# ORNL-Fusion/graph_framework

Measured on AMD Instinct MI355X. Metric: ray-steps/sec on xrays_bench cold-plasma; achieved HBM GB/s vs peak, higher is better.
Workload: dtype f64

## Files before the change

graph_framework_amd/build.py:

```python
import glob
import os
import subprocess

from . import _lib

HIPCC = os.environ.get("HIPCC", "/opt/rocm/bin/hipcc")
KERNEL_FLAGS = ["-O3", "-ffp-contract=off", "-fno-slp-vectorize", "--offload-arch=gfx950"]


def build_library(force=False):
    csrc = os.path.join(_lib.HERE, "csrc")
    sources = glob.glob(os.path.join(csrc, "*")) + glob.glob(os.path.join(_lib.HERE, "..", "include", "*.h"))
    newest = max(os.path.getmtime(s) for s in sources)
    programs = [os.path.join(_lib.HERE, name) for name in ("xrays_bench", "solver_check", "korc_push")]
    sources.append(os.path.join(_lib.HERE, "gf_workflow.hpp"))
    newest = max(os.path.getmtime(s) for s in sources)
    if (force or not os.path.exists(_lib.LIB_PATH) or os.path.getmtime(_lib.LIB_PATH) < newest
            or any(not os.path.exists(p) or os.path.getmtime(p) < newest for p in programs)):
        subprocess.check_call(["make", "-C", csrc, "-s", "HIPCC=" + HIPCC])
    return _lib.LIB_PATH


def compile_source(source, source_hash, force=False):
    os.makedirs(_lib.CACHE_DIR, exist_ok=True)
    stem = os.path.join(_lib.CACHE_DIR, "%016x" % source_hash)
    if force or not os.path.exists(stem + ".hsaco"):
        with open(stem + ".hip", "w") as f:
            f.write(source)
        subprocess.check_call([HIPCC, "--genco"] + KERNEL_FLAGS + ["-o", stem + ".hsaco", stem + ".hip"])
    return stem + ".hsaco"


LEVELS = (0, 1)


def prebuild_kernel(gfir_path, force=False):
    from . import backend
    return [compile_source(source, source_hash, force) for source, source_hash in backend.generate_piece_sources(gfir_path)]


VARIANTS = [({"GFHIP_DIVISION": "fast"}, "solver_kernel_f64"), ({"GFHIP_DIVISION": "fast"}, "loss_kernel_kx_f64"),
            ({"GFHIP_ASM": "0"}, "solver_kernel_f64"), ({"GFHIP_MERGE": "0"}, "solver_kernel_f64")]


def variant_sources():
    import json
    import sys
    texts = []
    for overrides, stem in VARIANTS:
        env = dict(os.environ)
        env.update(overrides)
        out = subprocess.run([sys.executable, "-c",
                              "import sys, json; sys.path.insert(0, %r)\n"
                              "from graph_framework_amd.backend import generate_piece_sources\n"
                              "print(json.dumps(generate_piece_sources(%r)))"
                              % (os.path.dirname(_lib.HERE), os.path.join(_lib.WORKLOAD_DIR, stem + ".gfir"))],
                             env=env, capture_output=True, text=True, check=True)
        texts += [tuple(piece) for piece in json.loads(out.stdout)]
    return texts


def prebuild_workloads(force=False):
    from concurrent.futures import ThreadPoolExecutor
    from . import backend
    paths = sorted(glob.glob(os.path.join(_lib.WORKLOAD_DIR, "*.gfir")))
    texts = [piece for path in paths for piece in backend.generate_piece_sources(path)] + variant_sources()
    known = {source_hash for _, source_hash in texts}
    for level in LEVELS[1:]:
        for path in paths:
            for piece in backend.generate_piece_sources(path, level):
                if piece[1] not in known:
                    known.add(piece[1])
                    texts.append(piece)
    workers = max(1, min(8, (os.cpu_count() or 4)))
    with ThreadPoolExecutor(max_workers=workers) as pool:
        built = list(pool.map(lambda piece: compile_source(piece[0], piece[1], force), texts))
    keep = {os.path.splitext(b)[0] for b in built}
    for stale in glob.glob(os.path.join(_lib.CACHE_DIR, "*")):
        if os.path.splitext(stale)[0] not in keep and not stale.endswith(".order"):
            os.remove(stale)
    return built


def build_all(force=False):
    build_library(force)
    return prebuild_workloads(force)
```

graph_framework_amd/csrc/asm_body.hpp:

```cpp
#ifndef gfhip_asm_body_hpp
#define gfhip_asm_body_hpp

#include <algorithm>
#include <cstdint>
#include <cstdio>
#include <cstdlib>
#include <cstring>
#include <map>
#include <set>
#include <sstream>
#include <string>
#include <tuple>
#include <vector>

#include "gfir_item.hpp"
#include "merge.hpp"
#include "options.hpp"
#include "schedule.hpp"
#include "tables.hpp"

namespace gfhip {

struct asm_body_text {
    bool ok = false;
    std::string why;
    std::string statement;
    uint32_t slots = 0;
    size_t vector = 0, scalar = 0, lds_reads = 0, lds_writes = 0, loads = 0, waits = 0;
    size_t signs_folded = 0, signs_kept = 0;
    size_t tables_folded = 0, tables_kept = 0;
    size_t twins_folded = 0, twins_made = 0;
};

class asm_body_writer {
    const item &it;
    const codegen_options &opt;
    const std::vector<pack> &packs;
    const std::vector<int> &parent;
    const std::vector<double> &factor;
    const std::vector<uint32_t> &table_pack, &table_column;
    const uint32_t block_size;
    const uint32_t slot_limit;

    static constexpr size_t never = static_cast<size_t> (1) << 60;
    static constexpr int sgpr_lo = 56, sgpr_pairs = 22;

    const size_t n = it.code.size();
    const uint32_t pool_lo, pairs;

    std::ostringstream a;
    asm_body_text result;

    struct value {
        int reg = -1;
        int slot = -1;
        bool defined = false;
        bool loadable = false;
        int64_t vm = -1, lgkm = -1;
        std::string operand;
        std::vector<size_t> uses;
        size_t cursor = 0;
        int group = -1;
        uint32_t table = 0;
    };
    std::vector<value> values;
    std::vector<int64_t> alias;
    std::vector<bool> negated;
    std::vector<bool> folded;
    std::vector<std::vector<int64_t>> used_at;
    std::vector<int64_t> owner;
    std::vector<int> free_slots;
    std::set<int64_t> pinned;
    size_t position = 0;

    struct group {
        int offset_pair = -1;
        uint32_t pack = 0;
        size_t last_use = 0;
        std::map<uint32_t, int64_t> cells;
    };
    typedef std::tuple<uint32_t, uint32_t, uint32_t, uint32_t, double, double, double, double> group_key;
    std::map<group_key, int> group_of_key;
    std::vector<group> groups;
    std::vector<int> node_group;

    int64_t vm_issued = 0, lgkm_issued = 0, vm_done = -1, lgkm_done = -1;

    struct constant_slot { uint64_t bits = 0; bool valid = false; size_t stamp = 0; };
    std::vector<constant_slot> constants = std::vector<constant_slot> (sgpr_pairs);
    size_t constant_clock = 0;

    int pending_track_pair = -1;

  public:
    asm_body_writer(const item &it_, const codegen_options &opt_, const std::vector<pack> &packs_, const std::vector<int> &parent_,
                    const std::vector<double> &factor_, const std::vector<uint32_t> &table_pack_,
                    const std::vector<uint32_t> &table_column_, const uint32_t block_size_, const uint32_t slot_limit_)
        : it(it_), opt(opt_), packs(packs_), parent(parent_), factor(factor_), table_pack(table_pack_), table_column(table_column_),
          block_size(block_size_), slot_limit(slot_limit_), pool_lo(opt_.asm_pool_lo & ~1u), pairs((256 - (opt_.asm_pool_lo & ~1u))/2) {}

    static std::string why_not(const item &it, const codegen_options &opt) {
        if (it.dtype != GFIR_F64) return "not an fp64 item";
        if (it.safe_math() || it.has_random()) return "SAFE_MATH or random draws";
        if (opt.division != division_mode::shared) return "division mode is not `shared`";
        if (opt.division_fixup == 1) return "v_div_fixup requested";
        for (size_t i = 0; i < it.code.size(); i++) {
            const gfir_instruction &c = it.code[i];
            switch (c.op) {
                case GFIR_CONST: case GFIR_INPUT: case GFIR_ADD: case GFIR_SUB: case GFIR_MUL: case GFIR_FMA: case GFIR_GATHER1: case GFIR_GATHER2:
                    break;
                case GFIR_POWI:
                    if (c.aux < 2) return "pow with an integer exponent below 2";
                    if (it.code[c.a].op == GFIR_CONST) return "power of a constant";
                    break;
                case GFIR_DIV:
                    if (it.code[c.b].op == GFIR_CONST) return "division by a constant";
                    break;
                case GFIR_SQRT:
                    if (it.code[c.a].op == GFIR_CONST) return "square root of a constant";
                    break;
                case GFIR_POW:
                    if (!(opt.pow_three_halves && it.code[c.b].op == GFIR_CONST && it.code[c.b].imm[0] == 1.5)) return "pow with an exponent other than 1.5";
                    if (it.code[c.a].op == GFIR_CONST) return "power of a constant";
                    break;
                default:
                    return "an operation without a sequence in asm_body.hpp";
            }
        }
        for (size_t i = 0; i < it.symbols.size(); i++) {
            if (it.indexed_length(static_cast<uint32_t> (i))) return "indexed inputs";
        }
        return "";
    }

  private:
    std::string note;
    void annotate(const std::string &text) { note = text; }
    void line(const std::string &text) {
        a << "                \"" << text;
        if (!note.empty()) a << " ; " << note;
        note.clear();
        a << "\\n\"\n";
    }
    std::string value_name(const int64_t id) const {
        if (id < static_cast<int64_t> (n)) return "r" + std::to_string(id);
        if (id < static_cast<int64_t> (2*n)) return "q" + std::to_string(id - static_cast<int64_t> (n));
        const value &v = values[static_cast<size_t> (id)];
        return "c" + std::to_string(v.group) + "_" + std::to_string(v.table);
    }
    void vector_op(const std::string &text) { line(text); result.vector++; }
    void scalar_op(const std::string &text) { line(text); result.scalar++; }
    static std::string pair_name(const int p, const uint32_t lo) {
        const uint32_t r = lo + 2u*static_cast<uint32_t> (p);
        return "v[" + std::to_string(r) + ":" + std::to_string(r + 1) + "]";
    }
    std::string pair_name(const int p) const { return pair_name(p, pool_lo); }
    std::string low_name(const int p) const { return "v" + std::to_string(pool_lo + 2u*static_cast<uint32_t> (p)); }
    std::string high_name(const int p) const { return "v" + std::to_string(pool_lo + 2u*static_cast<uint32_t> (p) + 1u); }
    static std::string hex32(const uint32_t v) {
        char buffer[16];
        std::snprintf(buffer, sizeof(buffer), "0x%x", v);
        return buffer;
    }

    size_t next_use(const int64_t id, const size_t from) {
        value &v = values[static_cast<size_t> (id)];
        while (v.cursor < v.uses.size() && v.uses[v.cursor] < from) v.cursor++;
        return v.cursor < v.uses.size() ? v.uses[v.cursor] : never;
    }
    void add_use(const int64_t id, const size_t at) {
        std::vector<size_t> &u = values[static_cast<size_t> (id)].uses;
        if (u.empty() || u.back() != at) u.push_back(at);
        if (at < n) {
            std::vector<int64_t> &here = used_at[at];
            if (std::find(here.begin(), here.end(), id) == here.end()) here.push_back(id);
        }
    }

    int64_t cell_value(const int g, const uint32_t t) {
        auto found = groups[static_cast<size_t> (g)].cells.find(t);
        if (found != groups[static_cast<size_t> (g)].cells.end()) return found->second;
        value v;
        v.loadable = true;
        v.group = g;
        v.table = t;
        values.push_back(v);
        const int64_t id = static_cast<int64_t> (values.size()) - 1;
        groups[static_cast<size_t> (g)].cells[t] = id;
        return id;
    }

    std::vector<bool> needs_register() const {
        std::vector<bool> needed(n, false);
        for (size_t i = 0; i < n; i++) {
            const gfir_instruction &c = it.code[i];
            if (it.is_merged(i)) continue;
            switch (c.op) {
                case GFIR_GATHER2: needed[c.b] = true; needed[c.a] = true; break;
                case GFIR_GATHER1: case GFIR_POWI: case GFIR_SQRT: case GFIR_POW: needed[c.a] = true; break;
                case GFIR_DIV: needed[c.b] = true; break;
                default: break;
            }
        }
        for (auto &st : it.setters) needed[st.value] = true;
        for (auto o : it.outputs) needed[o] = true;
        return needed;
    }
    static bool is_minus_one(const gfir_instruction &c) { return c.op == GFIR_CONST && c.imm[0] == -1.0 && c.imm[1] == 0.0; }

    void analyse() {
        values.assign(2*n, value());
        alias.assign(n, -1);
        negated.assign(n, false);
        folded.assign(n, false);
        const std::vector<bool> needed = opt.level >= 1 ? needs_register() : std::vector<bool> ();
        used_at.assign(n, std::vector<int64_t> ());
        node_group.assign(n, -1);
        for (size_t i = 0; i < n; i++) {
            const gfir_instruction &c = it.code[i];
            alias[i] = static_cast<int64_t> (i);
            if (c.op == GFIR_GATHER1 || c.op == GFIR_GATHER2) {
                const table &t = it.tables[c.aux];
                const bool two = c.op == GFIR_GATHER2;
                const group_key key(c.a, two ? c.b : GFIR_NONE, t.rows, t.cols, c.imm[0], c.imm[1], two ? c.imm[2] : 0.0, two ? c.imm[3] : 0.0);
                auto found = group_of_key.find(key);
                if (found == group_of_key.end()) {
                    group g;
                    g.pack = table_pack[c.aux];
                    groups.push_back(g);
                    found = group_of_key.insert({key, static_cast<int> (groups.size()) - 1}).first;
                }
                node_group[i] = found->second;
                if (opt.level >= 1 && !it.is_merged(i) && parent[c.aux] >= 0 && factor[c.aux] == -1.0) {
                    if (!needed[i]) {
                        alias[i] = cell_value(found->second, static_cast<uint32_t> (parent[c.aux]));
                        negated[i] = true;
                        result.tables_folded++;
                        continue;
                    }
                    result.tables_kept++;
                }
                alias[i] = cell_value(found->second, c.aux);
            } else if (opt.level >= 1 && c.op == GFIR_MUL && !it.is_merged(i) && is_minus_one(it.code[c.a]) != is_minus_one(it.code[c.b])) {
                const uint32_t x = is_minus_one(it.code[c.a]) ? c.b : c.a;
                if (it.code[x].op == GFIR_CONST) continue;
                if (needed[i]) {
                    result.signs_kept++;
                    continue;
                }
                alias[i] = alias[x];
                negated[i] = !negated[x];
                folded[i] = true;
                result.signs_folded++;
            }
        }
        std::vector<bool> group_seen(groups.size(), false);
        for (size_t i = 0; i < n; i++) {
            const gfir_instruction &c = it.code[i];
            if (c.op == GFIR_CONST || c.op == GFIR_INPUT || it.is_merged(i) || folded[i]) continue;
            if (c.op == GFIR_GATHER1 || c.op == GFIR_GATHER2) {
                const size_t g = static_cast<size_t> (node_group[i]);
                if (!group_seen[g]) {
                    group_seen[g] = true;
                    if (it.code[c.a].op != GFIR_CONST) add_use(alias[c.a], i);
                    if (c.op == GFIR_GATHER2 && it.code[c.b].op != GFIR_CONST) add_use(alias[c.b], i);
                }
                continue;
            }
            const uint32_t operands[3] = {c.a, c.b, c.c};
            for (int k = 0; k < operand_count(c.op); k++) {
                if (it.code[operands[k]].op != GFIR_CONST) add_use(alias[operands[k]], i);
            }
            if (c.op == GFIR_DIV) add_use(static_cast<int64_t> (n + c.b), i);
        }
        for (auto &st : it.setters) {
            if (it.code[st.value].op != GFIR_CONST) add_use(alias[st.value], n);
        }
        for (auto o : it.outputs) {
            if (it.code[o].op != GFIR_CONST) add_use(alias[o], n);
        }
        for (size_t k = 2*n; k < values.size(); k++) {
            int64_t child = static_cast<int64_t> (k);
            while (parent[values[static_cast<size_t> (child)].table] >= 0) {
                const int g = values[static_cast<size_t> (child)].group;
                const int64_t up = cell_value(g, static_cast<uint32_t> (parent[values[static_cast<size_t> (child)].table]));
                std::vector<size_t> merged = values[static_cast<size_t> (up)].uses;
                for (const size_t u : values[static_cast<size_t> (k)].uses) merged.push_back(u);
                std::sort(merged.begin(), merged.end());
                merged.erase(std::unique(merged.begin(), merged.end()), merged.end());
                values[static_cast<size_t> (up)].uses = merged;
                for (const size_t u : values[static_cast<size_t> (k)].uses) {
                    if (u < n && std::find(used_at[u].begin(), used_at[u].end(), up) == used_at[u].end()) used_at[u].push_back(up);
                }
                child = up;
            }
        }
        for (auto &g : groups) {
            for (auto &kv : g.cells) {
                for (const size_t u : values[static_cast<size_t> (kv.second)].uses) g.last_use = std::max(g.last_use, u);
            }
        }
    }

    bool in_flight(const value &v) const { return v.vm > vm_done || v.lgkm > lgkm_done; }

    void flush_track() {
        if (pending_track_pair < 0) return;
        const std::string h = "abs(" + high_name(pending_track_pair) + ")";
        vector_op("v_maximum3_f32 %[dmax], %[dmax], " + h + ", " + h);
        vector_op("v_minimum3_f32 %[dmin], %[dmin], " + h + ", " + h);
        pending_track_pair = -1;
    }
    void track(const int pair) {
        if (pending_track_pair < 0) {
            pending_track_pair = pair;
            return;
        }
        const std::string first = "abs(" + high_name(pending_track_pair) + ")", second = "abs(" + high_name(pair) + ")";
        vector_op("v_maximum3_f32 %[dmax], %[dmax], " + first + ", " + second);
        vector_op("v_minimum3_f32 %[dmin], %[dmin], " + first + ", " + second);
        pending_track_pair = -1;
    }

    void release_pair(const int p) {
        if (p == pending_track_pair) flush_track();
        owner[static_cast<size_t> (p)] = -1;
    }

    std::string slot_address(const int slot, std::string &base) const {
        const uint32_t per_base = 65536u/(block_size*8u);
        base = "%[park" + std::to_string(static_cast<uint32_t> (slot)/per_base) + "]";
        return std::to_string((static_cast<uint32_t> (slot)%per_base)*block_size*8u);
    }

    int take_pair(const size_t horizon = 0) {
        for (size_t p = 0; p < owner.size(); p++) {
            if (owner[p] == -1) {
                owner[p] = -2;
                return static_cast<int> (p);
            }
        }
        int best = -1;
        size_t farthest = 0;
        bool best_needs_slot = true;
        for (size_t p = 0; p < owner.size(); p++) {
            const int64_t id = owner[p];
            if (id < 0 || pinned.count(id)) continue;
            value &v = values[static_cast<size_t> (id)];
            if (in_flight(v)) continue;
            const size_t u = next_use(id, position);
            if (horizon && u <= horizon) continue;
            const bool needs_slot = !v.loadable && v.slot < 0 && v.operand.empty();
            if (needs_slot && free_slots.empty() && result.slots >= slot_limit) continue;
            if (best < 0 || u > farthest || (u == farthest && best_needs_slot && !needs_slot)) {
                best = static_cast<int> (p);
                farthest = u;
                best_needs_slot = needs_slot;
            }
        }
        if (best < 0) return -1;
        const int64_t id = owner[static_cast<size_t> (best)];
        value &v = values[static_cast<size_t> (id)];
        if (best == pending_track_pair) flush_track();
        if (!v.loadable && v.slot < 0) {
            if (free_slots.empty()) {
                v.slot = static_cast<int> (result.slots++);
            } else {
                v.slot = free_slots.back();
                free_slots.pop_back();
            }
            std::string base;
            const std::string offset = slot_address(v.slot, base);
            annotate("spill " + value_name(id));
            line("ds_write_b64 " + base + ", " + pair_name(best) + " offset:" + offset);
            lgkm_issued++;
            result.lds_writes++;
        }
        v.reg = -1;
        owner[static_cast<size_t> (best)] = -2;
        return best;
    }

    int need_pair() {
        const int p = take_pair();
        if (p < 0 && result.why.empty()) result.why = "the register pool and the LDS slots are both full";
        return p < 0 ? 0 : p;
    }

    void wait_for(value &v) {
        if (v.vm > vm_done) {
            const int64_t allowed = std::min<int64_t> (vm_issued - 1 - v.vm, 63);
            line("s_waitcnt vmcnt(" + std::to_string(allowed) + ")");
            vm_done = vm_issued - 1 - allowed;
            result.waits++;
        }
        if (v.lgkm > lgkm_done) {
            const int64_t allowed = std::min<int64_t> (lgkm_issued - 1 - v.lgkm, 15);
            line("s_waitcnt lgkmcnt(" + std::to_string(allowed) + ")");
            lgkm_done = lgkm_issued - 1 - allowed;
            result.waits++;
        }
    }

    bool fetch(const int64_t id, const size_t horizon = 0) {
        value &v = values[static_cast<size_t> (id)];
        if (v.reg >= 0 || !v.operand.empty()) return true;
        if (v.loadable) {
            const group &g = groups[static_cast<size_t> (v.group)];
            if (g.offset_pair < 0) return false;
            if (parent[v.table] >= 0) {
                if (horizon) return false;
                const int64_t up = cell_value(v.group, static_cast<uint32_t> (parent[v.table]));
// ... 257 lines not shown
        vector_op("v_fma_f64 " + E + ", -" + den + ", " + R + ", 1.0");
        annotate("def " + value_name(id));
        vector_op("v_fma_f64 " + R + ", " + R + ", " + E + ", " + R);
        release_pair(e);
        values[static_cast<size_t> (id)].reg = r;
        values[static_cast<size_t> (id)].defined = true;
        owner[static_cast<size_t> (r)] = id;
    }

    int square_root(const std::string &x, const std::string &defines = std::string()) {
        const int g = need_pair(), h = need_pair(), y = need_pair();
        const std::string G = pair_name(g), H = pair_name(h), Y = pair_name(y);
        vector_op("v_rsq_f64_e32 " + Y + ", " + x);
        line("s_nop 0");
        vector_op("v_mul_f64 " + G + ", " + x + ", " + Y);
        vector_op("v_mul_f64 " + H + ", " + Y + ", 0.5");
        vector_op("v_fma_f64 " + Y + ", -" + H + ", " + G + ", 0.5");
        vector_op("v_fma_f64 " + G + ", " + G + ", " + Y + ", " + G);
        vector_op("v_fma_f64 " + H + ", " + H + ", " + Y + ", " + H);
        vector_op("v_fma_f64 " + Y + ", -" + G + ", " + G + ", " + x);
        vector_op("v_fma_f64 " + G + ", " + Y + ", " + H + ", " + G);
        vector_op("v_fma_f64 " + Y + ", -" + G + ", " + G + ", " + x);
        if (!defines.empty()) annotate(defines);
        vector_op("v_fma_f64 " + G + ", " + Y + ", " + H + ", " + G);
        release_pair(h);
        release_pair(y);
        return g;
    }

    int in_pool(const uint32_t node, bool &copied) {
        value &v = values[static_cast<size_t> (alias[node])];
        copied = false;
        if (v.operand.empty()) return v.reg;
        const int p = need_pair();
        vector_op("v_mov_b64 " + pair_name(p) + ", " + v.operand);
        copied = true;
        return p;
    }

    void find_cell(const size_t i) {
        const gfir_instruction &c = it.code[i];
        group &g = groups[static_cast<size_t> (node_group[i])];
        const table &t = it.tables[c.aux];
        const bool two = c.op == GFIR_GATHER2;
        const pack &pk = packs[g.pack];
        const int dimensions = two ? 2 : 1;
        int quotient[2] = {-1, -1}, index[2] = {-1, -1};
        for (int d = 0; d < dimensions; d++) {
            const uint32_t arg = d == 0 ? c.a : c.b;
            const double scale = c.imm[2*d], offset = c.imm[2*d + 1];
            operands x = resolve({arg});
            const int q = need_pair(), e = need_pair();
            const std::string Q = pair_name(q), E = pair_name(e);
            int taken = -1;
            if (it.code[arg].op == GFIR_CONST) {
                vector_op("v_mov_b32_e32 " + low_name(e) + ", " + hex32(static_cast<uint32_t> (bits_of(it.code[arg].imm[0]))));
                vector_op("v_mov_b32_e32 " + high_name(e) + ", " + hex32(static_cast<uint32_t> (bits_of(it.code[arg].imm[0]) >> 32)));
                vector_op("v_add_f64 " + E + ", " + E + ", " + constant_operand(-offset, &taken));
            } else {
                vector_op("v_add_f64 " + E + ", " + x.text[0] + ", " + constant_operand(-offset, &taken));
            }
            done_with(x);
            const int m = need_pair();
            const std::string M = pair_name(m);
            taken = -1;
            vector_op("v_mul_f64 " + Q + ", " + E + ", " + constant_operand(1.0/scale, &taken));
            taken = -1;
            vector_op("v_fma_f64 " + M + ", " + constant_operand(-scale, &taken) + ", " + Q + ", " + E);
            taken = -1;
            vector_op("v_fma_f64 " + Q + ", " + M + ", " + constant_operand(1.0/scale, &taken) + ", " + Q);
            release_pair(m);
            release_pair(e);
            quotient[d] = q;
        }
        {
            const std::string first = "abs(" + high_name(quotient[0]) + ")", second = "abs(" + high_name(quotient[dimensions - 1]) + ")";
            vector_op("v_maximum3_f32 %[vmax], %[vmax], " + first + ", " + second);
        }
        for (int d = 0; d < dimensions; d++) {
            const uint32_t length = d == 0 ? (two ? t.rows : t.cols) : t.cols;
            const std::string Q = pair_name(quotient[d]);
            int taken = -1;
            vector_op("v_max_f64 " + Q + ", " + Q + ", 0");
            vector_op("v_min_f64 " + Q + ", " + Q + ", " + constant_operand(static_cast<double> (length - 1), &taken));
            vector_op("v_cvt_u32_f64_e32 " + low_name(quotient[d]) + ", " + Q);
            index[d] = quotient[d];
        }
        const int cell = index[0];
        if (two) {
            if (t.cols <= 64) {
                vector_op("v_mad_u32_u24 " + low_name(cell) + ", " + low_name(index[0]) + ", " + std::to_string(t.cols) + ", " + low_name(index[1]));
            } else {
                vector_op("v_mul_u32_u24_e32 " + low_name(cell) + ", " + hex32(t.cols) + ", " + low_name(index[0]));
                vector_op("v_add_u32_e32 " + low_name(cell) + ", " + low_name(cell) + ", " + low_name(index[1]));
            }
            release_pair(index[1]);
        }
        const std::string defines = "def g" + std::to_string(node_group[i]) + " node " + std::to_string(i) + " stride " + std::to_string(pk.stride*8u) +
                                    " pack " + std::to_string(g.pack) + " lds " + std::to_string(pk.in_lds ? 1 : 0);
        if (!pk.in_lds) annotate(defines);
        vector_op("v_mul_u32_u24_e32 " + low_name(cell) + ", " + hex32(pk.stride*8u) + ", " + low_name(cell));
        if (pk.in_lds) {
            annotate(defines);
            vector_op("v_add_u32_e32 " + low_name(cell) + ", %[lds" + std::to_string(g.pack) + "], " + low_name(cell));
        }
        g.offset_pair = cell;
        owner[static_cast<size_t> (cell)] = -2;
    }

    void node(const size_t i) {
        const gfir_instruction &c = it.code[i];
        position = i;
        pinned.clear();
        if (it.is_merged(i)) {
            line("; alias r" + std::to_string(i) + " = r" + std::to_string(it.merged_into[i]));
            return;
        }
        if (folded[i]) {
            line("; alias r" + std::to_string(i) + " = " + (negated[i] ? "-" : "") + value_name(alias[i]));
            return;
        }
        look_ahead();
        std::vector<int64_t> read = used_at[i];
        switch (c.op) {
            case GFIR_CONST:
                return;
            case GFIR_INPUT:
                values[i].operand = "%[v" + std::to_string(c.a) + "]";
                values[i].defined = true;
                return;
            case GFIR_GATHER1:
            case GFIR_GATHER2:
                if (groups[static_cast<size_t> (node_group[i])].offset_pair == -1) find_cell(i);
                line("; alias r" + std::to_string(i) + " = " + (negated[i] ? "-" : "") + value_name(alias[i]));
                break;
            case GFIR_ADD:
            case GFIR_SUB:
            case GFIR_MUL:
            case GFIR_FMA: {
                operands x = c.op == GFIR_FMA ? resolve({c.a, c.b, c.c}, {}, true) : resolve({c.a, c.b}, {false, c.op == GFIR_SUB}, true);
                retire(read);
                read.clear();
                const int p = need_pair();
                const char *name = c.op == GFIR_MUL ? "v_mul_f64 " : c.op == GFIR_FMA ? "v_fma_f64 " : "v_add_f64 ";
                std::string text = name + pair_name(p);
                for (auto &operand : x.text) text += ", " + operand;
                annotate("def r" + std::to_string(i));
                vector_op(text);
                done_with(x);
                define(i, p);
                break;
            }
            case GFIR_POWI: {
                operands x = resolve({c.a});
                const int p = need_pair();
                if (c.aux == 2) annotate("def r" + std::to_string(i));
                vector_op("v_mul_f64 " + pair_name(p) + ", " + x.text[0] + ", " + x.text[0]);
                for (uint32_t k = 2; k < c.aux; k++) {
                    if (k + 1 == c.aux) annotate("def r" + std::to_string(i));
                    vector_op("v_mul_f64 " + pair_name(p) + ", " + pair_name(p) + ", " + x.text[0]);
                }
                done_with(x);
                define(i, p);
                break;
            }
            case GFIR_DIV: {
                const int64_t r = static_cast<int64_t> (n + c.b);
                pinned.insert(r);
                operands x = resolve({c.a, c.b});
                if (!values[static_cast<size_t> (r)].defined) {
                    bool copied = false;
                    const int d = in_pool(c.b, copied);
                    track(d);
                    if (copied) {
                        flush_track();
                        release_pair(d);
                    }
                    reciprocal(c.b);
                } else {
                    fetch(r);
                    wait_for(values[static_cast<size_t> (r)]);
                }
                const std::string R = name_of(r);
                const int q = need_pair(), e = need_pair();
                const std::string Q = pair_name(q), E = pair_name(e);
                std::string negative_denominator = x.text[1][0] == '-' ? x.text[1].substr(1) : "-" + x.text[1];
                vector_op("v_mul_f64 " + Q + ", " + x.text[0] + ", " + R);
                vector_op("v_fma_f64 " + E + ", " + negative_denominator + ", " + Q + ", " + x.text[0]);
                annotate("def r" + std::to_string(i));
                vector_op("v_fma_f64 " + Q + ", " + E + ", " + R + ", " + Q);
                release_pair(e);
                done_with(x);
                define(i, q);
                break;
            }
            case GFIR_SQRT: {
                operands x = resolve({c.a});
                bool copied = false;
                const int argument = in_pool(c.a, copied);
                track(argument);
                const int p = square_root(pair_name(argument), "def r" + std::to_string(i));
                if (copied) {
                    flush_track();
                    release_pair(argument);
                }
                done_with(x);
                define(i, p);
                break;
            }
            case GFIR_POW: {
                operands x = resolve({c.a});
                bool copied = false;
                const int argument = in_pool(c.a, copied);
                track(argument);
                const std::string X = pair_name(argument);
                const int s = square_root(X);
                const int t = need_pair(), u = need_pair(), p = need_pair();
                const std::string S = pair_name(s), T = pair_name(t), U = pair_name(u), P = pair_name(p);
                vector_op("v_rcp_f64_e32 " + T + ", " + S);
                line("s_nop 0");
                vector_op("v_mul_f64 " + T + ", " + T + ", 0.5");
                vector_op("v_fma_f64 " + U + ", -" + S + ", " + S + ", " + X);
                vector_op("v_mul_f64 " + T + ", " + U + ", " + T);
                vector_op("v_mul_f64 " + P + ", " + X + ", " + S);
                vector_op("v_fma_f64 " + U + ", " + X + ", " + S + ", -" + P);
                vector_op("v_mul_f64 " + T + ", " + X + ", " + T);
                vector_op("v_add_f64 " + U + ", " + U + ", " + T);
                annotate("def r" + std::to_string(i));
                vector_op("v_add_f64 " + P + ", " + P + ", " + U);
                release_pair(s);
                release_pair(t);
                release_pair(u);
                if (copied) {
                    flush_track();
                    release_pair(argument);
                }
                done_with(x);
                define(i, p);
                break;
            }
            default:
                result.why = "an operation without a sequence in asm_body.hpp";
                return;
        }
        retire(read);
        for (auto &g : groups) {
            if (g.offset_pair >= 0 && g.last_use <= i) {
                release_pair(g.offset_pair);
                g.offset_pair = -2;
            }
        }
    }

  public:
    asm_body_text write() {
        result.why = why_not(it, opt);
        if (!result.why.empty()) return result;
        analyse();
        owner.assign(pairs, -1);
        line("s_waitcnt lgkmcnt(0)");
        for (size_t i = 0; i < n && result.why.empty(); i++) {
            node(i);
            if (std::getenv("GFHIP_ASM_TRACE") && (i%100 == 0 || !result.why.empty())) {
                size_t in_registers = 0, tables = 0, reciprocals = 0, parked = 0;
                for (size_t p = 0; p < owner.size(); p++) {
                    if (owner[p] == -1) continue;
                    in_registers++;
                    if (owner[p] >= static_cast<int64_t> (2*n)) tables++;
                    else if (owner[p] >= static_cast<int64_t> (n)) reciprocals++;
                }
                for (auto &v : values) parked += v.slot >= 0 && v.reg < 0;
                std::fprintf(stderr, "  node %zu: %zu pairs in use (%zu table values, %zu reciprocals), %zu values only in LDS, %zu slots taken\n",
                             i, in_registers, tables, reciprocals, parked, static_cast<size_t> (result.slots) - free_slots.size());
            }
        }
        if (!result.why.empty()) return result;
        position = n;
        pinned.clear();
        flush_track();
        std::vector<std::pair<std::string, uint32_t>> targets;
        for (size_t k = 0; k < it.setters.size(); k++) targets.push_back({"%[sv" + std::to_string(k) + "]", it.setters[k].value});
        for (size_t o = 0; o < it.outputs.size(); o++) targets.push_back({"%[so" + std::to_string(o) + "]", it.outputs[o]});
        std::map<uint32_t, int> staged;
        for (auto &target : targets) {
            const gfir_instruction &c = it.code[target.second];
            if (c.op == GFIR_CONST) continue;
            const int64_t id = alias[target.second];
            pinned.insert(id);
            if (!values[static_cast<size_t> (id)].operand.empty() && !staged.count(target.second)) {
                const int p = need_pair();
                vector_op("v_mov_b64 " + pair_name(p) + ", " + values[static_cast<size_t> (id)].operand);
                staged[target.second] = p;
            }
        }
        for (auto &target : targets) {
            const gfir_instruction &c = it.code[target.second];
            if (c.op == GFIR_CONST) {
                const uint64_t bits = bits_of(c.imm[0]);
                const int p = need_pair();
                vector_op("v_mov_b32_e32 " + low_name(p) + ", " + hex32(static_cast<uint32_t> (bits)));
                vector_op("v_mov_b32_e32 " + high_name(p) + ", " + hex32(static_cast<uint32_t> (bits >> 32)));
                annotate("out constant " + std::to_string(bits));
                vector_op("v_mov_b64 " + target.first + ", " + pair_name(p));
                release_pair(p);
                continue;
            }
            const int64_t id = alias[target.second];
            if (staged.count(target.second)) {
                annotate("out r" + std::to_string(target.second));
                vector_op("v_mov_b64 " + target.first + ", " + pair_name(staged[target.second]));
                continue;
            }
            fetch(id);
            wait_for(values[static_cast<size_t> (id)]);
            annotate("out r" + std::to_string(target.second));
            vector_op("v_mov_b64 " + target.first + ", " + name_of(id));
        }
        line("s_waitcnt vmcnt(0) lgkmcnt(0)");
        if (!result.why.empty()) return result;

        std::ostringstream s;
        s << "                asm volatile(\n" << a.str() << "                : ";
        bool first = true;
        auto separator = [&] () { if (!first) s << ", "; first = false; };
        for (size_t k = 0; k < it.setters.size(); k++) { separator(); s << "[sv" << k << "] \"=v\"(sv" << k << ")"; }
        for (size_t o = 0; o < it.outputs.size(); o++) { separator(); s << "[so" << o << "] \"=v\"(so" << o << ")"; }
        separator();
        s << "[dmax] \"+v\"(dmax), [dmin] \"+v\"(dmin), [vmax] \"+v\"(vmax)\n                : ";
        first = true;
        std::vector<bool> input_read(it.symbols.size(), false);
        for (size_t i = 0; i < n; i++) {
            if (it.code[i].op == GFIR_INPUT && !values[i].uses.empty()) input_read[it.code[i].a] = true;
        }
        for (size_t i = 0; i < it.symbols.size(); i++) {
            if (input_read[i]) { separator(); s << "[v" << i << "] \"v\"(v" << i << ")"; }
        }
        for (size_t p = 0; p < packs.size(); p++) {
            separator();
            if (packs[p].in_lds) s << "[lds" << p << "] \"v\"(lds_address" << p << ")";
            else s << "[pack" << p << "] \"s\"(pack" << p << ")";
        }
        if (result.slots) {
            separator();
            const uint32_t per_base = 65536u/(block_size*8u);
            for (uint32_t k = 0; k*per_base < result.slots; k++) {
                if (k) s << ", ";
                s << "[park" << k << "] \"v\"(park" << k << ")";
            }
        }
        s << "\n                : ";
        for (uint32_t r = pool_lo; r < 256; r++) s << "\"v" << r << "\", ";
        for (int r = sgpr_lo; r < sgpr_lo + 2*sgpr_pairs; r++) s << "\"s" << r << "\", ";
        s << "\"memory\");\n";
        result.statement = s.str();
        result.ok = true;
        return result;
    }
};

inline item schedule_for_assembly(const item &in, const codegen_options &opt, const std::vector<std::string> &directories = {}) {
    if (too_large_to_schedule(in) || !asm_body_writer::why_not(in, opt).empty()) return schedule_for_pressure(in);
    if (const char *forced = std::getenv("GFHIP_ASM_SEED")) {
        return reorder(in, list_schedule(in, static_cast<uint32_t> (std::atoi(forced))));
    }
    const std::vector<uint8_t> bytes = in.serialize();
    const uint64_t key = fnv1a(std::string(bytes.begin(), bytes.end()) + "|order|" + std::to_string(opt.asm_pool_lo) + "|" +
                               std::to_string(opt.asm_load_ahead) + "|" + std::to_string(opt.asm_reload_ahead) + "|" +
                               std::to_string(opt.asm_schedule_tries) + "|" + std::to_string(opt.asm_wide_loads) + "|" +
                               std::to_string(opt.lds_budget) + "|" + std::to_string(opt.compact_tables) + "|" + std::to_string(opt.block_size) +
                               (opt.merge ? "|merged" : ""));
    char name[40];
    std::snprintf(name, sizeof(name), "/%016llx.order", static_cast<unsigned long long> (key));
    for (auto &directory : directories) {
        if (FILE *f = std::fopen((directory + name).c_str(), "r")) {
            unsigned int seed = 0;
            const bool read = std::fscanf(f, "%u", &seed) == 1;
            std::fclose(f);
            if (read) return reorder(in, list_schedule(in, seed));
        }
    }
    const table_layout layout = layout_tables(in, opt);
    item best;
    uint32_t best_seed = 0;
    size_t best_slots = ~static_cast<size_t> (0), best_traffic = 0;
    const uint32_t tries = in.code.size() <= 5000 ? opt.asm_schedule_tries
                         : std::max<uint32_t> (4u, static_cast<uint32_t> (opt.asm_schedule_tries*5000ull/in.code.size()));
    for (uint32_t seed = 0; seed < std::max(1u, tries); seed++) {
        item candidate = reorder(in, list_schedule(in, seed));
        const item merged = opt.merge ? merge_records(candidate) : item();
        codegen_options plain = opt;
        plain.level = 0;
        asm_body_writer writer(opt.merge ? merged : candidate, plain, layout.packs, layout.parent, layout.factor, layout.table_pack, layout.table_column,
                               opt.block_size, 1u << 20);
        const asm_body_text text = writer.write();
        if (!text.ok) continue;
        const size_t traffic = text.lds_reads + text.lds_writes;
        if (std::getenv("GFHIP_ASM_REPORT")) {
            std::fprintf(stderr, "  order %u of %s: %u slots, %zu LDS reads, %zu LDS writes, %zu loads, %zu waits\n", seed, in.name.c_str(), text.slots,
                         text.lds_reads, text.lds_writes, text.loads, text.waits);
        }
        if (text.slots < best_slots || (text.slots == best_slots && traffic < best_traffic)) {
            best_slots = text.slots;
            best_traffic = traffic;
            best = std::move(candidate);
            best_seed = seed;
        }
    }
    if (best.code.empty()) return schedule_for_pressure(in);
    for (auto &directory : directories) {
        if (FILE *f = std::fopen((directory + name).c_str(), "w")) {
            std::fprintf(f, "%u\n", best_seed);
            std::fclose(f);
            break;
        }
    }
    return best;
}

inline bool assembly_candidate(const item &piece, const codegen_options &opt) {
    return opt.asm_body && !piece.code.empty() && piece.code.size() >= opt.asm_min_nodes && asm_body_writer::why_not(piece, opt).empty();
}

inline uint32_t assembly_slot_limit(const size_t lds_used, const codegen_options &opt, const size_t element_size) {
    const size_t per_block = 160u*1024u/opt.asm_waves;
    return lds_used < per_block ? static_cast<uint32_t> ((per_block - lds_used)/(static_cast<size_t> (opt.block_size)*element_size)) : 0;
}

inline asm_body_text assembly_statement(const item &piece, const codegen_options &opt) {
    const table_layout layout = layout_tables(piece, opt);
    const uint32_t slot_limit = assembly_slot_limit(layout.lds_used, opt, piece.element_size());
    auto write = [&] (const item &form, const codegen_options &options) {
        asm_body_writer writer(form, options, layout.packs, layout.parent, layout.factor, layout.table_pack, layout.table_column, options.block_size,
                               slot_limit);
        return writer.write();
    };
    auto report = [&] (const asm_body_text &text, const char *what) {
        if (!std::getenv("GFHIP_ASM_REPORT")) return;
        std::fprintf(stderr, "assembly body of %s%s: %s; %zu vector, %zu scalar, %zu table loads, %zu LDS reads, %zu LDS writes, %zu waits, %u slots\n",
                     piece.name.c_str(), what, text.ok ? "ok" : text.why.c_str(), text.vector, text.scalar, text.loads,
                     text.lds_reads, text.lds_writes, text.waits, text.slots);
    };
    codegen_options plain = opt;
    plain.level = 0;
    const asm_body_text text = write(piece, plain);
    report(text, "");
    if (opt.level < 1 || !text.ok) return text;
    merge_report merges;
    const item again = opt.merge ? merge_records(piece, &merges, opt.level) : item();
    const asm_body_text folded = write(opt.merge ? again : piece, opt);
    report(folded, " (level 1)");
    if (std::getenv("GFHIP_ASM_REPORT")) {
        if (opt.merge) merges.print(stderr, piece.name + " (level 1)");
        std::fprintf(stderr, "level 1 folds of %s: mul by -1.0: %zu folded, %zu kept; gathers of a table derived by -1.0: %zu folded, %zu kept; "
                             "-k*p read from the register of k*p: %zu times, multiplied all the same: %zu times; %zu vector instructions fewer\n",
                     piece.name.c_str(), folded.signs_folded, folded.signs_kept, folded.tables_folded, folded.tables_kept, folded.twins_folded,
                     folded.twins_made, text.vector - folded.vector);
    }
    return folded.ok ? folded : text;
}

}

#endif
```

graph_framework_amd/csrc/options.hpp:

```cpp
#ifndef gfhip_options_hpp
#define gfhip_options_hpp

#include <cstdint>
#include <cstdlib>
#include <string>

namespace gfhip {

enum class division_mode {
    shared,
    checked,
    ieee,
    fast
};

struct codegen_options {
    size_t lds_budget = 64*1024;
    uint32_t block_size = 256;
    uint32_t waves_per_simd = 0;
    division_mode division = division_mode::shared;
    bool pow_three_halves = true;
    bool window_sqrt = false;
    bool window_sqrt_f32 = true;
    int nontemporal = -1;
    bool compact_tables = true;
    bool park_in_lds = true;
    uint32_t park_min_range = 1500;
    uint32_t park_window = 100;
    uint32_t park_max_slots = 32;
    uint32_t park_prefetch = 50;
    uint32_t park_capacity = 0;
    bool schedule_for_pressure = true;
    int division_fixup = -1;
    uint32_t converge_batch = 3;
    uint32_t segment_nodes = 6000;
    uint32_t segments = 0;
    uint32_t segments_min_nodes = 2000;
    bool asm_body = true;
    uint32_t asm_waves = 2;
    bool asm_wide_loads = true;
    uint32_t asm_schedule_tries = 64;
    uint32_t asm_min_nodes = 1000;
    uint32_t asm_pool_lo = 40;
    uint32_t asm_load_ahead = 96;
    uint32_t asm_reload_ahead = 24;
    bool merge = true;
    uint32_t level = 0;
    size_t handover_bytes = 128u << 20;

    static codegen_options from_environment(const uint32_t level = 0) {
        codegen_options o;
        o.level = level;
        if (const char *e = std::getenv("GFHIP_LEVEL")) o.level = std::atoi(e) > 0 ? 1 : 0;
        if (const char *e = std::getenv("GFHIP_DIVISION")) {
            const std::string mode(e);
            o.division = mode == "ieee" ? division_mode::ieee : mode == "checked" ? division_mode::checked
                       : mode == "fast" ? division_mode::fast : division_mode::shared;
        }
        if (const char *e = std::getenv("GFHIP_PARK")) {
            const std::string mode(e);
            o.park_in_lds = mode != "0";
            if (mode == "heavy") o.park_min_range = 300;
        }
        if (const char *e = std::getenv("GFHIP_SCHEDULE")) o.schedule_for_pressure = std::string(e) != "source";
        if (const char *e = std::getenv("GFHIP_DIV_FIXUP")) o.division_fixup = std::string(e) != "0" ? 1 : 0;
        if (const char *e = std::getenv("GFHIP_NONTEMPORAL")) o.nontemporal = std::atoi(e);
        if (const char *e = std::getenv("GFHIP_COMPACT_TABLES")) o.compact_tables = std::string(e) != "0";
        if (const char *e = std::getenv("GFHIP_POW")) o.pow_three_halves = std::string(e) != "libm";
        if (const char *e = std::getenv("GFHIP_PARK_CAPACITY")) o.park_capacity = static_cast<uint32_t> (std::atoi(e));
        if (const char *e = std::getenv("GFHIP_PARK_PREFETCH")) o.park_prefetch = static_cast<uint32_t> (std::atoi(e));
        if (const char *e = std::getenv("GFHIP_ASM")) o.asm_body = std::string(e) != "0";
        if (const char *e = std::getenv("GFHIP_ASM_WAVES")) o.asm_waves = static_cast<uint32_t> (std::atoi(e)) == 2 ? 2 : 1;
        if (const char *e = std::getenv("GFHIP_ASM_WIDE_LOADS")) o.asm_wide_loads = std::string(e) != "0";
        if (const char *e = std::getenv("GFHIP_ASM_TRIES")) o.asm_schedule_tries = static_cast<uint32_t> (std::atoi(e));
        if (const char *e = std::getenv("GFHIP_ASM_MIN_NODES")) o.asm_min_nodes = static_cast<uint32_t> (std::atoi(e));
        if (const char *e = std::getenv("GFHIP_ASM_POOL_LO")) o.asm_pool_lo = static_cast<uint32_t> (std::atoi(e));
        if (const char *e = std::getenv("GFHIP_ASM_LOAD_AHEAD")) o.asm_load_ahead = static_cast<uint32_t> (std::atoi(e));
        if (const char *e = std::getenv("GFHIP_ASM_RELOAD_AHEAD")) o.asm_reload_ahead = static_cast<uint32_t> (std::atoi(e));
        if (const char *e = std::getenv("GFHIP_WINDOW_SQRT")) o.window_sqrt = std::string(e) == "1";
        if (const char *e = std::getenv("GFHIP_WINDOW_SQRT_F32")) o.window_sqrt_f32 = std::string(e) == "1";
        if (const char *e = std::getenv("GFHIP_WAVES_PER_SIMD")) o.waves_per_simd = static_cast<uint32_t> (std::atoi(e));
        if (const char *e = std::getenv("GFHIP_LDS_BUDGET")) o.lds_budget = static_cast<size_t> (std::atol(e));
        if (const char *e = std::getenv("GFHIP_CONVERGE_BATCH")) o.converge_batch = static_cast<uint32_t> (std::atol(e) > 0 ? std::atol(e) : 1);
        if (o.converge_batch > 8) o.converge_batch = 8;
        if (const char *e = std::getenv("GFHIP_SEGMENT_NODES")) o.segment_nodes = static_cast<uint32_t> (std::atol(e));
        if (const char *e = std::getenv("GFHIP_SEGMENTS")) o.segments = static_cast<uint32_t> (std::atol(e));
        if (const char *e = std::getenv("GFHIP_SEGMENTS_MIN_NODES")) o.segments_min_nodes = static_cast<uint32_t> (std::atol(e));
        if (const char *e = std::getenv("GFHIP_MERGE")) o.merge = std::string(e) != "0";
        if (const char *e = std::getenv("GFHIP_HANDOVER_BYTES")) o.handover_bytes = static_cast<size_t> (std::atoll(e));
        return o;
    }
};

inline uint64_t fnv1a(const std::string &s) {
    uint64_t h = 1469598103934665603ull;
    for (unsigned char c : s) {
        h ^= c;
        h *= 1099511628211ull;
    }
    return h;
}

inline const char *compile_flags() {
    return "-O3 -ffp-contract=off -fno-slp-vectorize --offload-arch=gfx950";
}

}

#endif
```

graph_framework_amd/csrc/solver_check.cpp:

```cpp
#include <cstdio>
#include <cstdlib>

#include "../gf_workflow.hpp"

int main(int argc, char **argv) {
    if (argc != 8) {
        std::fprintf(stderr, "usage: solver_check <workload directory> <prefix> <omega> <kx> <ky> <kz> <steps>\n");
        return 2;
    }
    const size_t steps = std::strtoull(argv[7], nullptr, 10);
    gf::solver::ray_solver<double> solve(argv[1], argv[2], 1);
    solve.state["w"][0] = std::atof(argv[3]);
    solve.state["kx"][0] = std::atof(argv[4]);
    solve.state["ky"][0] = std::atof(argv[5]);
    solve.state["kz"][0] = std::atof(argv[6]);

    const double tolerance = 1.0E-30;
    solve.init("kx", tolerance);
    solve.sync_host();
    auto print = [&] (const double residual) {
        for (const char *name : {"t", "w", "x", "y", "z", "kx", "ky", "kz"}) std::printf("%.17g ", solve.state[name][0]);
        std::printf("%.17g\n", residual);
    };
    std::printf("newton_iterations %zu\n", solve.newton_iterations);
    print(solve.newton_residual(0));
    solve.solver_level = 1;
    solve.compile();
    bool holds = true;
    for (size_t i = 0; i < steps; i++) {
        solve.step();
        const double residual = solve.check_residual(0);
        holds = holds && std::abs(residual) < std::abs(tolerance);
        solve.sync_host();
        print(residual);
    }
    std::printf("holds %d\n", holds ? 1 : 0);
    return 0;
}
```

graph_framework_amd/csrc/xrays_bench.cpp:

```cpp
#include <algorithm>
#include <chrono>
#include <cstdio>
#include <cstdlib>
#include <fstream>
#include <iostream>
#include <string>
#include <thread>
#include <vector>

#include "../gf_workflow.hpp"

namespace {

struct threaded_timer {
    std::string label;
    std::vector<double> seconds;
    std::vector<std::chrono::steady_clock::time_point> starts;
    threaded_timer(const std::string &l, const size_t threads) : label(l), seconds(threads, 0.0), starts(threads) {}
    void start_time(const size_t i) { starts[i] = std::chrono::steady_clock::now(); }
    void end_time(const size_t i) {
        seconds[i] = std::chrono::duration<double> (std::chrono::steady_clock::now() - starts[i]).count();
    }
    void print() const {
        double sum = 0.0, longest = 0.0;
        for (double s : seconds) { sum += s; longest = std::max(longest, s); }
        std::printf("%-14s: average %.6f s  max %.6f s\n", label.c_str(), sum/static_cast<double> (seconds.size()), longest);
    }
};

}

int main(int argc, char **argv) {
    if (argc < 2) {
        std::cerr << "usage: xrays_bench <workload directory> [num_rays] [num_times]" << std::endl;
        return 2;
    }
    const std::string directory = argv[1];
    const size_t num_rays = argc > 2 ? strtoull(argv[2], nullptr, 10) : 100000;
    const size_t num_times = argc > 3 ? strtoull(argv[3], nullptr, 10) : 1000;
    const std::string output_prefix = argc > 4 ? argv[4] : "";
    const size_t sub_steps = argc > 5 ? strtoull(argv[5], nullptr, 10) : 100;

    const size_t devices = static_cast<size_t> (std::max(gfhip_max_concurrency(), 0));
    if (devices == 0) {
        std::cerr << "no HIP device" << std::endl;
        return 1;
    }
    std::vector<std::thread> threads(std::max<size_t> (std::min(devices, num_rays), 1));
    const size_t batch = num_rays/threads.size();
    const size_t extra = num_rays%threads.size();

    threaded_timer time_setup("Setup Time", threads.size()), time_init("Init Time", threads.size());
    threaded_timer time_compile("Compile Time", threads.size()), time_steps("Time Steps", threads.size());
    std::vector<double> final_x(threads.size()), final_kx(threads.size()), residual(threads.size());
    std::vector<size_t> iterations(threads.size());

    std::cout << gfhip_device_type() << ", " << threads.size() << " device thread(s), " << num_rays << " rays, "
              << num_times << " steps" << std::endl;

    for (size_t i = 0, ie = threads.size(); i < ie; i++) {
        threads[i] = std::thread([&, i] () {
            time_setup.start_time(i);
            const size_t local_num_rays = batch + (extra > i ? 1 : 0);
            size_t first = 0, last = 0;
            if (gfhip_shard_bounds(num_rays, threads.size(), i, &first, &last) || last - first != local_num_rays) {
                std::cerr << "shard split disagrees with xrays_bench.cpp:38-51" << std::endl;
                exit(1);
            }
            gf::solver::ray_solver<double> solve(directory, "", local_num_rays, i);
            solve.state["w"].assign(local_num_rays, 500.0);
            solve.state["x"].assign(local_num_rays, 2.5);
            solve.state["kx"].assign(local_num_rays, -600.0);
            time_setup.end_time(i);

            time_init.start_time(i);
            solve.init("kx");
            iterations[i] = solve.newton_iterations;
            time_init.end_time(i);

            time_compile.start_time(i);
            solve.solver_level = 1;
            solve.compile();
            time_compile.end_time(i);

            if (!output_prefix.empty()) {
                solve.open_result_file(output_prefix + std::to_string(i) + ".nc");
                solve.write_step();
            }
            time_steps.start_time(i);
            for (size_t j = 0; j < num_times; j++) {
                solve.step();
                if (!output_prefix.empty() && sub_steps && (j + 1)%sub_steps == 0) solve.write_step();
            }
            solve.sync_host();
            time_steps.end_time(i);
            solve.close_result_file();

            final_x[i] = solve.state["x"][local_num_rays - 1];
            final_kx[i] = solve.state["kx"][local_num_rays - 1];
            residual[i] = solve.check_residual(0);
        });
    }
    for (std::thread &t : threads) {
        t.join();
    }

    time_setup.print();
    time_init.print();
    time_compile.print();
    time_steps.print();
    double slowest = 0.0;
    for (double s : time_steps.seconds) slowest = std::max(slowest, s);
    std::printf("ray-steps/s (max over devices, step loop + sync_host): %.6e\n",
                static_cast<double> (num_rays)*static_cast<double> (num_times)/slowest);
    for (size_t i = 0; i < threads.size(); i++) {
        std::printf("device %zu: Newton iterations %zu, x = %.17g, kx = %.17g, residual = %.17g\n",
                    i, iterations[i], final_x[i], final_kx[i], residual[i]);
    }
    return 0;
}
```

Baseline: 5.896 billion.

## Add level-2 asm folds reusing sqrt, squares and implied reciprocals

Adds a level-2 codegen pass in the asm body writer. It reuses an earlier sqrt of the same argument for pow(x,1.5), builds powi(x,p>=3) from an existing x*x record, and computes denominators implied by a tracked root or power through a reciprocal path instead of a full division. The benchmark and solver check now compile at level 2, and the build prebuilds level-2 kernels. This cuts redundant f64 sqrt, multiply and divide sequences in the ray solver kernel, at the cost of longer value live ranges and more register pressure, and it can change rounding.

```diff
diff --git a/graph_framework_amd/build.py b/graph_framework_amd/build.py
--- a/graph_framework_amd/build.py
+++ b/graph_framework_amd/build.py
@@ -31,7 +31,7 @@
     return stem + ".hsaco"
 
 
-LEVELS = (0, 1)
+LEVELS = (0, 1, 2)
 
 
 def prebuild_kernel(gfir_path, force=False):
diff --git a/graph_framework_amd/csrc/asm_body.hpp b/graph_framework_amd/csrc/asm_body.hpp
--- a/graph_framework_amd/csrc/asm_body.hpp
+++ b/graph_framework_amd/csrc/asm_body.hpp
@@ -30,6 +30,10 @@
     size_t signs_folded = 0, signs_kept = 0;
     size_t tables_folded = 0, tables_kept = 0;
     size_t twins_folded = 0, twins_made = 0;
+    size_t pow_sites = 0, pow_folded = 0, pow_kept_later = 0, pow_kept_none = 0;
+    size_t powi_sites = 0, powi_folded = 0, powi_kept = 0;
+    size_t windows = 0, windows_by_root = 0, windows_by_power = 0;
+    size_t windows_kept_input = 0, windows_kept_root = 0;
 };
 
 class asm_body_writer {
@@ -67,6 +71,9 @@
     std::vector<int64_t> alias;
     std::vector<bool> negated;
     std::vector<bool> folded;
+    std::vector<int64_t> root_of;
+    std::vector<int64_t> square_of;
+    std::vector<int64_t> implied_by;
     std::vector<std::vector<int64_t>> used_at;
     std::vector<int64_t> owner;
     std::vector<int> free_slots;
@@ -208,6 +215,97 @@
     }
     static bool is_minus_one(const gfir_instruction &c) { return c.op == GFIR_CONST && c.imm[0] == -1.0 && c.imm[1] == 0.0; }
 
+    void analyse_reuse() {
+        std::map<int64_t, size_t> first_root, first_square;
+        std::set<int64_t> any_root, root_argument;
+        std::vector<std::pair<int64_t, uint32_t>> power(n, {-1, 0});
+        auto plain = [this] (const uint32_t o) { return it.code[o].op != GFIR_CONST && !negated[o]; };
+        for (size_t i = 0; i < n; i++) {
+            const gfir_instruction &c = it.code[i];
+            if (c.op == GFIR_SQRT && !it.is_merged(i) && plain(c.a)) any_root.insert(alias[c.a]);
+            if ((c.op == GFIR_SQRT || c.op == GFIR_POW) && !it.is_merged(i) && it.code[c.a].op != GFIR_CONST) root_argument.insert(alias[c.a]);
+        }
+        for (size_t i = 0; i < n; i++) {
+            const gfir_instruction &c = it.code[i];
+            if (it.is_merged(i) || folded[i]) continue;
+            switch (c.op) {
+                case GFIR_SQRT:
+                    if (plain(c.a)) first_root.insert({alias[c.a], i});
+                    break;
+                case GFIR_POW: {
+                    result.pow_sites++;
+                    auto found = plain(c.a) ? first_root.find(alias[c.a]) : first_root.end();
+                    if (found != first_root.end()) {
+                        root_of[i] = static_cast<int64_t> (found->second);
+                        result.pow_folded++;
+                    } else if (plain(c.a) && any_root.count(alias[c.a])) {
+                        result.pow_kept_later++;
+                    } else {
+                        result.pow_kept_none++;
+                    }
+                    break;
+                }
+                case GFIR_POWI:
+                    if (!plain(c.a) || c.aux < 2) break;
+                    power[i] = {alias[c.a], c.aux};
+                    if (c.aux == 2) {
+                        first_square.insert({alias[c.a], i});
+                        break;
+                    }
+                    result.powi_sites++;
+                    if (first_square.count(alias[c.a])) {
+                        square_of[i] = static_cast<int64_t> (first_square[alias[c.a]]);
+                        result.powi_folded++;
+                    } else {
+                        result.powi_kept++;
+                    }
+                    break;
+                case GFIR_MUL:
+                    if (!plain(c.a) || !plain(c.b)) break;
+                    if (alias[c.a] == alias[c.b]) {
+                        power[i] = {alias[c.a], 2};
+                        first_square.insert({alias[c.a], i});
+                    } else if (alias[c.a] < static_cast<int64_t> (n) && power[static_cast<size_t> (alias[c.a])].first == alias[c.b]) {
+                        power[i] = {alias[c.b], power[static_cast<size_t> (alias[c.a])].second + 1};
+                    }
+                    break;
+                default:
+                    break;
+            }
+        }
+        std::vector<bool> denominator(n, false);
+        for (size_t i = 0; i < n; i++) {
+            if (it.code[i].op == GFIR_DIV && !it.is_merged(i)) denominator[it.code[i].b] = true;
+        }
+        std::map<int64_t, std::vector<size_t>> powers_of;
+        for (size_t d = n; d-- > 0;) {
+            if (!denominator[d]) continue;
+            result.windows++;
+            const gfir_instruction &c = it.code[d];
+            int64_t implier = -1;
+            if (c.op == GFIR_SQRT && it.code[c.a].op != GFIR_CONST) {
+                implier = static_cast<int64_t> (c.a);
+            } else if (!negated[d]) {
+                auto found = powers_of.find(alias[d]);
+                if (found != powers_of.end()) implier = static_cast<int64_t> (found->second.front());
+            }
+            if (implier >= 0 && root_argument.count(alias[d])) {
+                result.windows_kept_root++;
+                implier = -1;
+            }
+            if (implier >= 0 && c.op == GFIR_INPUT) {
+                result.windows_kept_input++;
+                implier = -1;
+            }
+            if (implier >= 0) {
+                implied_by[d] = implier;
+                (c.op == GFIR_SQRT ? result.windows_by_root : result.windows_by_power)++;
+                continue;
+            }
+            if (power[d].first >= 0) powers_of[power[d].first].push_back(d);
+        }
+    }
+
     void analyse() {
         values.assign(2*n, value());
         alias.assign(n, -1);
@@ -254,10 +352,16 @@
                 result.signs_folded++;
             }
         }
+        root_of.assign(n, -1);
+        square_of.assign(n, -1);
+        implied_by.assign(n, -1);
+        if (opt.level >= 2) analyse_reuse();
         std::vector<bool> group_seen(groups.size(), false);
         for (size_t i = 0; i < n; i++) {
             const gfir_instruction &c = it.code[i];
             if (c.op == GFIR_CONST || c.op == GFIR_INPUT || it.is_merged(i) || folded[i]) continue;
+            if (root_of[i] >= 0) add_use(root_of[i], i);
+            if (square_of[i] >= 0) add_use(square_of[i], i);
             if (c.op == GFIR_GATHER1 || c.op == GFIR_GATHER2) {
                 const size_t g = static_cast<size_t> (node_group[i]);
                 if (!group_seen[g]) {
@@ -821,6 +925,20 @@
                 break;
             }
             case GFIR_POWI: {
+                if (square_of[i] >= 0) {
+                    operands x = resolve({c.a, static_cast<uint32_t> (square_of[i])});
+                    const int p = need_pair();
+                    line("; alias square of r" + std::to_string(i) + " = r" + std::to_string(square_of[i]));
+                    if (c.aux == 3) annotate("def r" + std::to_string(i));
+                    vector_op("v_mul_f64 " + pair_name(p) + ", " + x.text[1] + ", " + x.text[0]);
+                    for (uint32_t k = 3; k < c.aux; k++) {
+                        if (k + 1 == c.aux) annotate("def r" + std::to_string(i));
+                        vector_op("v_mul_f64 " + pair_name(p) + ", " + pair_name(p) + ", " + x.text[0]);
+                    }
+                    done_with(x);
+                    define(i, p);
+                    break;
+                }
                 operands x = resolve({c.a});
                 const int p = need_pair();
                 if (c.aux == 2) annotate("def r" + std::to_string(i));
@@ -837,7 +955,10 @@
                 const int64_t r = static_cast<int64_t> (n + c.b);
                 pinned.insert(r);
                 operands x = resolve({c.a, c.b});
-                if (!values[static_cast<size_t> (r)].defined) {
+                if (!values[static_cast<size_t> (r)].defined && implied_by[c.b] >= 0) {
+                    line("; implied r" + std::to_string(c.b) + " " + name_of(alias[c.b]) + " by r" + std::to_string(implied_by[c.b]));
+                    reciprocal(c.b);
+                } else if (!values[static_cast<size_t> (r)].defined) {
                     bool copied = false;
                     const int d = in_pool(c.b, copied);
                     track(d);
@@ -878,14 +999,20 @@
                 break;
             }
             case GFIR_POW: {
-                operands x = resolve({c.a});
+                const bool reuse = root_of[i] >= 0;
+                operands x = reuse ? resolve({c.a, static_cast<uint32_t> (root_of[i])}) : resolve({c.a});
                 bool copied = false;
-                const int argument = in_pool(c.a, copied);
-                track(argument);
-                const std::string X = pair_name(argument);
-                const int s = square_root(X);
+                int argument = -1, s = -1;
+                if (reuse) {
+                    line("; alias s of r" + std::to_string(i) + " = r" + std::to_string(root_of[i]));
+                } else {
+                    argument = in_pool(c.a, copied);
+                    track(argument);
+                }
+                const std::string X = reuse ? x.text[0] : pair_name(argument);
+                if (!reuse) s = square_root(X);
                 const int t = need_pair(), u = need_pair(), p = need_pair();
-                const std::string S = pair_name(s), T = pair_name(t), U = pair_name(u), P = pair_name(p);
+                const std::string S = reuse ? x.text[1] : pair_name(s), T = pair_name(t), U = pair_name(u), P = pair_name(p);
                 vector_op("v_rcp_f64_e32 " + T + ", " + S);
                 line("s_nop 0");
                 vector_op("v_mul_f64 " + T + ", " + T + ", 0.5");
@@ -897,7 +1024,7 @@
                 vector_op("v_add_f64 " + U + ", " + U + ", " + T);
                 annotate("def r" + std::to_string(i));
                 vector_op("v_add_f64 " + P + ", " + P + ", " + U);
-                release_pair(s);
+                if (!reuse) release_pair(s);
                 release_pair(t);
                 release_pair(u);
                 if (copied) {
@@ -1117,7 +1244,18 @@
     merge_report merges;
     const item again = opt.merge ? merge_records(piece, &merges, opt.level) : item();
     const asm_body_text folded = write(opt.merge ? again : piece, opt);
-    report(folded, " (level 1)");
+    report(folded, opt.level >= 2 ? " (level 2)" : " (level 1)");
+    if (std::getenv("GFHIP_ASM_REPORT") && opt.level >= 2) {
+        std::fprintf(stderr, "level 2 folds of %s: pow(x, 1.5): %zu found, %zu take s from the sqrt record of x, %zu kept (sqrt record later in the "
+                             "order: %zu, no sqrt record of x: %zu); powi(x, p >= 3) not from its prefix: %zu found, %zu start from the record of "
+                             "x*x, %zu kept (no such record precedes it); denominators: %zu found, %zu not tracked (a sqrt record: %zu, the base of "
+                             "a tracked power: %zu), %zu kept (an input of the statement: %zu, a root argument as well: %zu, no tracked value implies it: %zu)\n",
+                     piece.name.c_str(), folded.pow_sites, folded.pow_folded, folded.pow_kept_later + folded.pow_kept_none, folded.pow_kept_later,
+                     folded.pow_kept_none, folded.powi_sites, folded.powi_folded, folded.powi_kept, folded.windows,
+                     folded.windows_by_root + folded.windows_by_power, folded.windows_by_root, folded.windows_by_power,
+                     folded.windows - folded.windows_by_root - folded.windows_by_power, folded.windows_kept_input, folded.windows_kept_root,
+                     folded.windows - folded.windows_by_root - folded.windows_by_power - folded.windows_kept_input - folded.windows_kept_root);
+    }
     if (std::getenv("GFHIP_ASM_REPORT")) {
         if (opt.merge) merges.print(stderr, piece.name + " (level 1)");
         std::fprintf(stderr, "level 1 folds of %s: mul by -1.0: %zu folded, %zu kept; gathers of a table derived by -1.0: %zu folded, %zu kept; "
diff --git a/graph_framework_amd/csrc/options.hpp b/graph_framework_amd/csrc/options.hpp
--- a/graph_framework_amd/csrc/options.hpp
+++ b/graph_framework_amd/csrc/options.hpp
@@ -51,7 +51,8 @@
     static codegen_options from_environment(const uint32_t level = 0) {
         codegen_options o;
         o.level = level;
-        if (const char *e = std::getenv("GFHIP_LEVEL")) o.level = std::atoi(e) > 0 ? 1 : 0;
+        if (const char *e = std::getenv("GFHIP_LEVEL")) o.level = std::atoi(e) > 0 ? static_cast<uint32_t> (std::atoi(e)) : 0;
+        if (o.level > 2) o.level = 2;
         if (const char *e = std::getenv("GFHIP_DIVISION")) {
             const std::string mode(e);
             o.division = mode == "ieee" ? division_mode::ieee : mode == "checked" ? division_mode::checked
diff --git a/graph_framework_amd/csrc/solver_check.cpp b/graph_framework_amd/csrc/solver_check.cpp
--- a/graph_framework_amd/csrc/solver_check.cpp
+++ b/graph_framework_amd/csrc/solver_check.cpp
@@ -24,7 +24,7 @@
     };
     std::printf("newton_iterations %zu\n", solve.newton_iterations);
     print(solve.newton_residual(0));
-    solve.solver_level = 1;
+    solve.solver_level = 2;
     solve.compile();
     bool holds = true;
     for (size_t i = 0; i < steps; i++) {
diff --git a/graph_framework_amd/csrc/xrays_bench.cpp b/graph_framework_amd/csrc/xrays_bench.cpp
--- a/graph_framework_amd/csrc/xrays_bench.cpp
+++ b/graph_framework_amd/csrc/xrays_bench.cpp
@@ -79,7 +79,7 @@
             time_init.end_time(i);
 
             time_compile.start_time(i);
-            solve.solver_level = 1;
+            solve.solver_level = 2;
             solve.compile();
             time_compile.end_time(i);
 
```

New measurement: 5.874 billion. No clear change (-0.4%).
